# run-house/kubetorch

Measured on NVIDIA H100. Metric: parallel_map_arg_plus_result_GBps, higher is better.
Workload: dtype f32

## Files before the change

### kubetorch_b200/csrc/ktb_map.cu

```cuda
#include "ktb_common.cuh"

#include <algorithm>
#include <atomic>

namespace ktb {

extern int g_red_ctas_per_sm;
extern int g_red_loads;
extern int g_red_fold;
extern int g_seg_large;
extern int g_mlp_chunk_rows;
}
extern int g_mlp_stage_ce;
namespace ktb {
extern std::atomic<int> g_host_zero_copy;
}
extern std::atomic<int> g_push_scatter_ctas_per_sm;
extern std::atomic<int> g_push_slice;
namespace ktb {

static std::atomic<int> g_vec_ctas_per_sm{0};
static std::atomic<int> g_tma_ctas_per_sm{1};
static std::atomic<int> g_tma_cfg{0};
static std::atomic<int> g_auto_variant{KTB_VARIANT_VEC};
static std::atomic<int> g_vec_flavor{2};
static std::atomic<int> g_vec_unroll{4};

constexpr int kVecThreads = 256;
constexpr int kVecUnroll = 4;
constexpr int kVecFlavor = 2;

template <int VB, int FL>
__device__ __forceinline__ void ld_vec(const uint8_t* p, uint32_t (&w)[VB / 4]) {
  static_assert(VB == 16, "sm_90 has no wider per-thread global access than 128 bits");
  if constexpr (FL == 1) {
    asm volatile("ld.global.v4.b32 {%0,%1,%2,%3}, [%4];"
                 : "=r"(w[0]), "=r"(w[1]), "=r"(w[2]), "=r"(w[3])
                 : "l"(p)
                 : "memory");
  } else if constexpr (FL == 2 || FL == 3) {
    ldg128_stream(p, w);
  } else {
    ldg128(p, w);
  }
}
template <int VB, int FL>
__device__ __forceinline__ void st_vec(uint8_t* p, const uint32_t (&w)[VB / 4]) {
  static_assert(VB == 16, "sm_90 has no wider per-thread global access than 128 bits");
  if constexpr (FL == 1) {
    asm volatile("st.global.v4.b32 [%0], {%1,%2,%3,%4};" ::"l"(p), "r"(w[0]), "r"(w[1]), "r"(w[2]), "r"(w[3])
                 : "memory");
  } else if constexpr (FL == 2) {
    stg128_stream(p, w);
  } else {
    stg128(p, w);
  }
}

template <int DT, int OP, int VB, int FL = kVecFlavor, int UNROLL = kVecUnroll>
__global__ void __launch_bounds__(kVecThreads)
    map_vec_kernel(const uint8_t* src, uint8_t* dst, size_t n_bytes, MapParams p) {
  constexpr int NW = VB / 4;
  constexpr int kVecUnroll = UNROLL;
  constexpr size_t TILE = (size_t)kVecThreads * kVecUnroll * VB;
  constexpr size_t ROW = (size_t)kVecThreads * VB;
  const size_t n_full = n_bytes / TILE;

  for (size_t t = blockIdx.x; t < n_full; t += gridDim.x) {
    const size_t off = t * TILE + (size_t)threadIdx.x * VB;
    uint32_t w[kVecUnroll][NW];
#pragma unroll
    for (int j = 0; j < kVecUnroll; ++j) ld_vec<VB, FL>(src + off + j * ROW, w[j]);
#pragma unroll
    for (int j = 0; j < kVecUnroll; ++j) {
      apply_words<DT, OP, NW>(w[j], p);
      st_vec<VB, FL>(dst + off + j * ROW, w[j]);
    }
  }

// ... 76 lines not shown
        }
        fence_proxy_async_smem();
        __syncthreads();
      }
      if (threadIdx.x == 0) {
        bulk_s2g(dst + tile_off(k), buf + (size_t)s * STAGE_BYTES, len);
        bulk_commit();
        if (k >= 1 && (k - 1 + STAGES) < my_n) {
          bulk_wait_read<1>();
          const size_t kn = k - 1 + STAGES;
          const int sn = (int)((k - 1) % STAGES);
          const uint32_t ln = tile_len(kn);
          mbar_expect_tx(&full[sn], ln);
          bulk_g2s(buf + (size_t)sn * STAGE_BYTES, src + tile_off(kn), ln, &full[sn]);
        }
      }
    }
    if (threadIdx.x == 0) bulk_wait_all<0>();
  }

  if (blockIdx.x == 0) {
    constexpr size_t ES = (DT == KTB_U8) ? 1 : ((DT == KTB_BF16 || DT == KTB_F16) ? 2 : (DT == KTB_I64 ? 8 : 4));
    const size_t n_tail = (n_bytes - n16) / ES;
    for (size_t e = threadIdx.x; e < n_tail; e += NT)
      apply_elem<DT, OP>(src + n16 + e * ES, dst + n16 + e * ES, p);
  }
}

template <int DT, int OP>
static int launch_typed(int dev, const uint8_t* src, uint8_t* dst, size_t n_elems, size_t es,
                        const MapParams& p, int variant, cudaStream_t stream) {
  const DeviceInfo* di = device_info(dev);
  const size_t n_bytes = n_elems * es;
  const uintptr_t both = (uintptr_t)src | (uintptr_t)dst;

  if (variant == KTB_VARIANT_AUTO) variant = g_auto_variant.load();
  if (variant == KTB_VARIANT_TMA && (both & 15)) variant = KTB_VARIANT_VEC;
  if (variant == KTB_VARIANT_VEC && (both & 15)) variant = KTB_VARIANT_SCALAR;

  if (variant == KTB_VARIANT_VEC) {
    const int per_sm = g_vec_ctas_per_sm.load();
    auto grid_for = [&](size_t tile_bytes) {
      size_t tiles = std::max<size_t>(n_bytes / tile_bytes, 1);
      if (per_sm <= 0) return (int)std::min<size_t>(tiles, 0x7fffffffULL);
      return (int)std::min<size_t>(tiles, (size_t)di->sm_count * per_sm);
    };
    constexpr bool kTunable = (DT == KTB_U8) || (DT == KTB_F32 && OP == KTB_OP_SCALE);
    const int fl = kTunable ? g_vec_flavor.load() : kVecFlavor;
    const int un = kTunable ? g_vec_unroll.load() : kVecUnroll;
#define KTB_VEC16(FL, UN)                                                                          \
  map_vec_kernel<DT, OP, 16, FL, UN>                                                               \
      <<<grid_for((size_t)kVecThreads * (UN)*16), kVecThreads, 0, stream>>>(src, dst, n_bytes, p)
    if constexpr (kTunable) {
      if (un == 2) {
        if (fl == 1) KTB_VEC16(1, 2); else if (fl == 2) KTB_VEC16(2, 2); else if (fl == 3) KTB_VEC16(3, 2); else KTB_VEC16(0, 2);
      } else if (un == 8) {
        if (fl == 1) KTB_VEC16(1, 8); else if (fl == 2) KTB_VEC16(2, 8); else if (fl == 3) KTB_VEC16(3, 8); else KTB_VEC16(0, 8);
      } else {
        if (fl == 1) KTB_VEC16(1, 4); else if (fl == 2) KTB_VEC16(2, 4); else if (fl == 3) KTB_VEC16(3, 4); else KTB_VEC16(0, 4);
      }
    } else {
      (void)fl; (void)un;
      KTB_VEC16(kVecFlavor, kVecUnroll);
    }
#undef KTB_VEC16
  } else if (variant == KTB_VARIANT_TMA) {
    const int cfg = g_tma_cfg.load();
    const int per_sm = std::max(1, g_tma_ctas_per_sm.load());
#define KTB_LAUNCH_TMA(ST, SB, NT)                                                              \
  do {                                                                                          \
    constexpr size_t smem_bytes = (size_t)(ST) * (SB) + (ST) * sizeof(uint64_t);                \
    auto kfn = map_tma_kernel<DT, OP, ST, SB, NT>;                                              \
    KTB_CK(cudaFuncSetAttribute(kfn, cudaFuncAttributeMaxDynamicSharedMemorySize,               \
                                (int)smem_bytes));                                              \
    size_t tiles = ((n_bytes & ~(size_t)15) + (SB)-1) / (SB);                                   \
    int grid = (int)std::min<size_t>(std::max<size_t>(tiles, 1), (size_t)di->sm_count * per_sm); \
    kfn<<<grid, NT, smem_bytes, stream>>>(src, dst, n_bytes, p);                                \
  } while (0)
    if (cfg == 1) {
      KTB_LAUNCH_TMA(6, 32768, 256);
    } else if (cfg == 2) {
      KTB_LAUNCH_TMA(6, 16384, 256);
    } else if (cfg == 3) {
      KTB_LAUNCH_TMA(3, 65536, 512);
    } else {
      KTB_LAUNCH_TMA(4, 32768, 256);
    }
#undef KTB_LAUNCH_TMA
  } else if (variant == KTB_VARIANT_SCALAR) {
    size_t blocks = (n_elems + 255) / 256;
    int grid = (int)std::min<size_t>(std::max<size_t>(blocks, 1), (size_t)di->sm_count * 8);
    map_scalar_kernel<DT, OP><<<grid, 256, 0, stream>>>(src, dst, n_elems, p);
  } else {
    set_error("ktb_map: unknown variant %d", variant);
    return KTB_ERR_ARG;
  }
  KTB_CK(cudaGetLastError());
  return KTB_OK;
}

int launch_map(int dev, int op, int dtype, const void* src_, void* dst_, size_t n_elems,
               const MapParams& p, int variant, cudaStream_t stream) {
  const uint8_t* src = static_cast<const uint8_t*>(src_);
  uint8_t* dst = static_cast<uint8_t*>(dst_);
  const size_t es = dtype_size(dtype);
  KTB_REQUIRE(es != 0, KTB_ERR_ARG, "ktb_map: unknown dtype %d", dtype);
  KTB_REQUIRE(op >= KTB_OP_IDENTITY && op <= KTB_OP_AFFINE, KTB_ERR_ARG, "ktb_map: unknown op %d", op);
  KTB_REQUIRE(!(dtype == KTB_U8 && op != KTB_OP_IDENTITY), KTB_ERR_ARG,
              "ktb_map: KTB_U8 supports KTB_OP_IDENTITY only");
  if (n_elems == 0) return KTB_OK;
  KTB_REQUIRE(src && dst, KTB_ERR_ARG, "ktb_map: null src/dst with n_elems=%zu", n_elems);
  KTB_REQUIRE((((uintptr_t)src | (uintptr_t)dst) & (es - 1)) == 0, KTB_ERR_ARG,
              "ktb_map: src/dst not aligned to the element size %zu", es);
  KTB_REQUIRE(n_elems <= (SIZE_MAX / 8), KTB_ERR_ARG, "ktb_map: n_elems too large");
  if (src != dst) {
    const uint8_t* se = src + n_elems * es;
    const uint8_t* de = dst + n_elems * es;
    KTB_REQUIRE(se <= dst || de <= src, KTB_ERR_ARG, "ktb_map: src and dst partially overlap");
  }

  if (op == KTB_OP_IDENTITY)
    return launch_typed<KTB_U8, KTB_OP_IDENTITY>(dev, src, dst, n_elems * es, 1, p, variant, stream);

#define KTB_CASE(DT)                                                                              \
  case DT:                                                                                        \
    return (op == KTB_OP_SCALE)                                                                   \
               ? launch_typed<DT, KTB_OP_SCALE>(dev, src, dst, n_elems, es, p, variant, stream)   \
               : launch_typed<DT, KTB_OP_AFFINE>(dev, src, dst, n_elems, es, p, variant, stream);
  switch (dtype) {
    KTB_CASE(KTB_F32)
    KTB_CASE(KTB_BF16)
    KTB_CASE(KTB_I32)
    KTB_CASE(KTB_I64)
    KTB_CASE(KTB_F16)
  }
#undef KTB_CASE
  set_error("ktb_map: unsupported dtype/op %d/%d", dtype, op);
  return KTB_ERR_UNSUPPORTED;
}

}

using namespace ktb;

extern "C" {

int ktb_set_tuning(int key, int value) {
  switch (key) {
    case 0: g_vec_ctas_per_sm = value; return KTB_OK;
    case 1: g_tma_ctas_per_sm = value; return KTB_OK;
    case 2: g_tma_cfg = value; return KTB_OK;
    case 4: g_vec_flavor = value; return KTB_OK;
    case 5: g_vec_unroll = value; return KTB_OK;
    case 6: g_red_ctas_per_sm = value > 0 ? value : 4; return KTB_OK;
    case 12: g_seg_large = value ? 1 : 0; return KTB_OK;
    case 13: g_red_loads = value == 4 ? 4 : 8; return KTB_OK;
    case 14: g_red_fold = value ? 1 : 0; return KTB_OK;
    case 20: g_host_zero_copy = value ? 1 : 0; return KTB_OK;
    case 23: g_push_slice = value > 0 ? value : 1; return KTB_OK;
    case 22: g_mlp_stage_ce = value ? 1 : 0; return KTB_OK;
    case 21: g_push_scatter_ctas_per_sm = value > 0 ? value : 0; return KTB_OK;
    case 8:
      KTB_REQUIRE(value > 0 && value % 128 == 0, KTB_ERR_ARG, "ktb_set_tuning: MLP chunk rows must be a multiple of 128");
      g_mlp_chunk_rows = value;
      return KTB_OK;
    case 3:
      KTB_REQUIRE(value >= KTB_VARIANT_VEC && value <= KTB_VARIANT_SCALAR, KTB_ERR_ARG,
                  "ktb_set_tuning: bad auto variant %d", value);
      g_auto_variant = value;
      return KTB_OK;
    default: set_error("ktb_set_tuning: unknown key %d", key); return KTB_ERR_ARG;
  }
}

int ktb_map(int dev, int op, int dtype, const void* src, void* dst, size_t n_elems, double alpha,
            double beta, int variant, uintptr_t stream) {
  int rc = require_device(dev);
  if (rc) return rc;
  KTB_GUARD(dev);
  return launch_map(dev, op, dtype, src, dst, n_elems, make_params(alpha, beta, dtype), variant,
                    reinterpret_cast<cudaStream_t>(stream));
}

int ktb_map_identity_u8(int dev, const void* src, void* dst, size_t nbytes, uintptr_t stream) {
  return ktb_map(dev, KTB_OP_IDENTITY, KTB_U8, src, dst, nbytes, 1.0, 0.0, KTB_VARIANT_AUTO, stream);
}
int ktb_map_scale_f32(int dev, const float* src, float* dst, size_t n, float alpha, uintptr_t stream) {
  return ktb_map(dev, KTB_OP_SCALE, KTB_F32, src, dst, n, alpha, 0.0, KTB_VARIANT_AUTO, stream);
}
int ktb_map_affine_f32(int dev, const float* src, float* dst, size_t n, float alpha, float beta,
                       uintptr_t stream) {
  return ktb_map(dev, KTB_OP_AFFINE, KTB_F32, src, dst, n, alpha, beta, KTB_VARIANT_AUTO, stream);
}
int ktb_map_scale_bf16(int dev, const void* src, void* dst, size_t n, float alpha, uintptr_t stream) {
  return ktb_map(dev, KTB_OP_SCALE, KTB_BF16, src, dst, n, alpha, 0.0, KTB_VARIANT_AUTO, stream);
}
int ktb_map_affine_bf16(int dev, const void* src, void* dst, size_t n, float alpha, float beta,
                        uintptr_t stream) {
  return ktb_map(dev, KTB_OP_AFFINE, KTB_BF16, src, dst, n, alpha, beta, KTB_VARIANT_AUTO, stream);
}

}
```

### kubetorch_b200/csrc/ktb_mlp.cu

```cuda
#include "ktb_common.cuh"

#include <cuda.h>
#include <algorithm>
#include <atomic>
#include <mutex>

namespace ktb {

constexpr int kMlpBlockM = 128;
constexpr int kMlpBlockK = 64;
constexpr int kMlpWgmmaK = 16;
constexpr int kMlpStages = 4;
constexpr int kMlpConsumers = 256;
constexpr int kMlpThreads = kMlpConsumers + 32;
int g_mlp_chunk_rows = 16896;

__device__ __forceinline__ void tma_load_2d(void* smem_dst, const CUtensorMap* map, int c0, int c1, uint64_t* bar) {
  asm volatile(
      "cp.async.bulk.tensor.2d.shared::cluster.global.mbarrier::complete_tx::bytes [%0], [%1, {%3, %4}], [%2];" ::
          "r"(smem_u32(smem_dst)),
      "l"(map), "r"(smem_u32(bar)), "r"(c0), "r"(c1)
      : "memory");
}
__device__ __forceinline__ void prefetch_tensormap(const CUtensorMap* map) {
  asm volatile("prefetch.tensormap [%0];" ::"l"(map) : "memory");
}
__device__ __forceinline__ void mbar_arrive(uint64_t* bar) {
  asm volatile("mbarrier.arrive.shared::cta.b64 _, [%0];" ::"r"(smem_u32(bar)) : "memory");
}
__device__ __forceinline__ void wgmma_fence() { asm volatile("wgmma.fence.sync.aligned;" ::: "memory"); }
__device__ __forceinline__ void wgmma_commit() { asm volatile("wgmma.commit_group.sync.aligned;" ::: "memory"); }
__device__ __forceinline__ void wgmma_wait_all() { asm volatile("wgmma.wait_group.sync.aligned 0;" ::: "memory"); }

__device__ __forceinline__ uint64_t make_smem_desc_sw128(const void* smem_tile) {
  const uint32_t addr = smem_u32(smem_tile);
  uint64_t d = 0;
  d |= (uint64_t)((addr & 0x3FFFFu) >> 4);
  d |= (uint64_t)1 << 16;
  d |= (uint64_t)(1024u >> 4) << 32;
  d |= (uint64_t)1 << 62;
  return d;
}

template <int N>
struct Wgmma;
template <>
struct Wgmma<256> {
  __device__ __forceinline__ static void mma(float (&d)[128], uint64_t adesc, uint64_t bdesc, uint32_t scale_d) {
    asm volatile(
        "{\n"
        ".reg .pred p;\n"
        "setp.ne.b32 p, %130, 0;\n"
        "wgmma.mma_async.sync.aligned.m64n256k16.f32.bf16.bf16 "
        "{%0,%1,%2,%3,%4,%5,%6,%7,%8,%9,%10,%11,%12,%13,%14,%15,%16,%17,%18,%19,%20,%21,%22,%23,%24,%25,%26,%27,%28,%29,%30,%31,%32,%33,%34,%35,%36,%37,%38,%39,%40,%41,%42,%43,%44,%45,%46,%47,%48,%49,%50,%51,%52,%53,%54,%55,%56,%57,%58,%59,%60,%61,%62,%63,%64,%65,%66,%67,%68,%69,%70,%71,%72,%73,%74,%75,%76,%77,%78,%79,%80,%81,%82,%83,%84,%85,%86,%87,%88,%89,%90,%91,%92,%93,%94,%95,%96,%97,%98,%99,%100,%101,%102,%103,%104,%105,%106,%107,%108,%109,%110,%111,%112,%113,%114,%115,%116,%117,%118,%119,%120,%121,%122,%123,%124,%125,%126,%127}, "
        "%128, %129, p, 1, 1, 0, 0;\n"
        "}\n"
        : "+f"(d[0]), "+f"(d[1]), "+f"(d[2]), "+f"(d[3]), "+f"(d[4]), "+f"(d[5]), "+f"(d[6]), "+f"(d[7]), "+f"(d[8]), "+f"(d[9]), "+f"(d[10]), "+f"(d[11]), "+f"(d[12]), "+f"(d[13]), "+f"(d[14]), "+f"(d[15]), "+f"(d[16]), "+f"(d[17]), "+f"(d[18]), "+f"(d[19]), "+f"(d[20]), "+f"(d[21]), "+f"(d[22]), "+f"(d[23]), "+f"(d[24]), "+f"(d[25]), "+f"(d[26]), "+f"(d[27]), "+f"(d[28]), "+f"(d[29]), "+f"(d[30]), "+f"(d[31]), "+f"(d[32]), "+f"(d[33]), "+f"(d[34]), "+f"(d[35]), "+f"(d[36]), "+f"(d[37]), "+f"(d[38]), "+f"(d[39]), "+f"(d[40]), "+f"(d[41]), "+f"(d[42]), "+f"(d[43]), "+f"(d[44]), "+f"(d[45]), "+f"(d[46]), "+f"(d[47]), "+f"(d[48]), "+f"(d[49]), "+f"(d[50]), "+f"(d[51]), "+f"(d[52]), "+f"(d[53]), "+f"(d[54]), "+f"(d[55]), "+f"(d[56]), "+f"(d[57]), "+f"(d[58]), "+f"(d[59]), "+f"(d[60]), "+f"(d[61]), "+f"(d[62]), "+f"(d[63]), "+f"(d[64]), "+f"(d[65]), "+f"(d[66]), "+f"(d[67]), "+f"(d[68]), "+f"(d[69]), "+f"(d[70]), "+f"(d[71]), "+f"(d[72]), "+f"(d[73]), "+f"(d[74]), "+f"(d[75]), "+f"(d[76]), "+f"(d[77]), "+f"(d[78]), "+f"(d[79]), "+f"(d[80]), "+f"(d[81]), "+f"(d[82]), "+f"(d[83]), "+f"(d[84]), "+f"(d[85]), "+f"(d[86]), "+f"(d[87]), "+f"(d[88]), "+f"(d[89]), "+f"(d[90]), "+f"(d[91]), "+f"(d[92]), "+f"(d[93]), "+f"(d[94]), "+f"(d[95]), "+f"(d[96]), "+f"(d[97]), "+f"(d[98]), "+f"(d[99]), "+f"(d[100]), "+f"(d[101]), "+f"(d[102]), "+f"(d[103]), "+f"(d[104]), "+f"(d[105]), "+f"(d[106]), "+f"(d[107]), "+f"(d[108]), "+f"(d[109]), "+f"(d[110]), "+f"(d[111]), "+f"(d[112]), "+f"(d[113]), "+f"(d[114]), "+f"(d[115]), "+f"(d[116]), "+f"(d[117]), "+f"(d[118]), "+f"(d[119]), "+f"(d[120]), "+f"(d[121]), "+f"(d[122]), "+f"(d[123]), "+f"(d[124]), "+f"(d[125]), "+f"(d[126]), "+f"(d[127])
        : "l"(adesc), "l"(bdesc), "r"(scale_d));
  }
};

template <>
struct Wgmma<64> {
  __device__ __forceinline__ static void mma(float (&d)[32], uint64_t adesc, uint64_t bdesc, uint32_t scale_d) {
    asm volatile(
        "{\n"
        ".reg .pred p;\n"
        "setp.ne.b32 p, %34, 0;\n"
        "wgmma.mma_async.sync.aligned.m64n64k16.f32.bf16.bf16 "
        "{%0,%1,%2,%3,%4,%5,%6,%7,%8,%9,%10,%11,%12,%13,%14,%15,%16,%17,%18,%19,%20,%21,%22,%23,%24,%25,%26,%27,%28,%29,%30,%31}, "
        "%32, %33, p, 1, 1, 0, 0;\n"
        "}\n"
        : "+f"(d[0]), "+f"(d[1]), "+f"(d[2]), "+f"(d[3]), "+f"(d[4]), "+f"(d[5]), "+f"(d[6]), "+f"(d[7]), "+f"(d[8]), "+f"(d[9]), "+f"(d[10]), "+f"(d[11]), "+f"(d[12]), "+f"(d[13]), "+f"(d[14]), "+f"(d[15]), "+f"(d[16]), "+f"(d[17]), "+f"(d[18]), "+f"(d[19]), "+f"(d[20]), "+f"(d[21]), "+f"(d[22]), "+f"(d[23]), "+f"(d[24]), "+f"(d[25]), "+f"(d[26]), "+f"(d[27]), "+f"(d[28]), "+f"(d[29]), "+f"(d[30]), "+f"(d[31])
        : "l"(adesc), "l"(bdesc), "r"(scale_d));
  }
};
template <int BLOCK_N, int STAGES>
struct MlpSmem {
  static constexpr int kABytes = kMlpBlockM * kMlpBlockK * 2;
  static constexpr int kBBytes = BLOCK_N * kMlpBlockK * 2;
  static constexpr int kStageBytes = kABytes + kBBytes;
  static constexpr int kBarrierOff = STAGES * kStageBytes;
  static constexpr int kTotal = kBarrierOff + 2 * STAGES * 8 + 1024 ;
};

template <int BLOCK_N, int STAGES, bool RELU>
__global__ void __launch_bounds__(kMlpThreads, 1)
    gemm_bf16_tn_wgmma_kernel(const __grid_constant__ CUtensorMap map_a, const __grid_constant__ CUtensorMap map_b,
                              __nv_bfloat16* __restrict__ C, int ldc, int K) {
  using S = MlpSmem<BLOCK_N, STAGES>;
  extern __shared__ uint8_t smem_raw[];
  uint8_t* smem = reinterpret_cast<uint8_t*>((reinterpret_cast<uintptr_t>(smem_raw) + 1023) & ~(uintptr_t)1023);
  uint64_t* full = reinterpret_cast<uint64_t*>(smem + S::kBarrierOff);
  uint64_t* empty = full + STAGES;

  const int warp = threadIdx.x >> 5;
  const int lane = threadIdx.x & 31;
  const int n0 = blockIdx.x * BLOCK_N;
  const int m0 = blockIdx.y * kMlpBlockM;
  const int num_kb = K / kMlpBlockK;

  if (threadIdx.x == 0) {
#pragma unroll
    for (int s = 0; s < STAGES; ++s) {
      mbar_init(&full[s], 1);
      mbar_init(&empty[s], kMlpConsumers);
    }
    fence_barrier_init();
  }
  __syncthreads();

  if (warp == kMlpConsumers / 32) {
    if (lane == 0) {
      prefetch_tensormap(&map_a);
      prefetch_tensormap(&map_b);
      for (int kb = 0; kb < num_kb; ++kb) {
        const int s = kb % STAGES;
        mbar_wait(&empty[s], ((kb / STAGES) & 1) ^ 1);
        uint8_t* a_dst = smem + (size_t)s * S::kStageBytes;
        mbar_expect_tx(&full[s], S::kStageBytes);
        tma_load_2d(a_dst, &map_a, kb * kMlpBlockK, m0, &full[s]);
        tma_load_2d(a_dst + S::kABytes, &map_b, kb * kMlpBlockK, n0, &full[s]);
      }
    }
    return;
  }

  const int wg = warp >> 2;
  float acc[BLOCK_N / 2];
#pragma unroll
  for (int i = 0; i < BLOCK_N / 2; ++i) acc[i] = 0.f;
  for (int kb = 0; kb < num_kb; ++kb) {
    const int s = kb % STAGES;
    mbar_wait(&full[s], (kb / STAGES) & 1);
    const uint8_t* a_src = smem + (size_t)s * S::kStageBytes + wg * 64 * 128;
    const uint64_t adesc = make_smem_desc_sw128(a_src);
    const uint64_t bdesc = make_smem_desc_sw128(smem + (size_t)s * S::kStageBytes + S::kABytes);
    wgmma_fence();
#pragma unroll
    for (int k = 0; k < kMlpBlockK / kMlpWgmmaK; ++k) {
      Wgmma<BLOCK_N>::mma(acc, adesc + (uint64_t)(2 * k), bdesc + (uint64_t)(2 * k), (uint32_t)((kb | k) != 0));
    }
    wgmma_commit();
    wgmma_wait_all();
    mbar_arrive(&empty[s]);
  }

  const int row = m0 + wg * 64 + (warp & 3) * 16 + (lane >> 2);
  __nv_bfloat16* c0 = C + (size_t)row * ldc + n0 + 2 * (lane & 3);
  __nv_bfloat16* c1 = c0 + (size_t)8 * ldc;
#pragma unroll
  for (int j = 0; j < BLOCK_N / 8; ++j) {
    float v[4] = {acc[4 * j], acc[4 * j + 1], acc[4 * j + 2], acc[4 * j + 3]};
    if (RELU) {
#pragma unroll
      for (int q = 0; q < 4; ++q) v[q] = fmaxf(v[q], 0.f);
    }
    *reinterpret_cast<__nv_bfloat162*>(c0 + 8 * j) = __floats2bfloat162_rn(v[0], v[1]);
    *reinterpret_cast<__nv_bfloat162*>(c1 + 8 * j) = __floats2bfloat162_rn(v[2], v[3]);
  }
}

typedef CUresult (*PFN_tensorMapEncodeTiled)(CUtensorMap*, CUtensorMapDataType, cuuint32_t, void*, const cuuint64_t*,
                                             const cuuint64_t*, const cuuint32_t*, const cuuint32_t*,
                                             CUtensorMapInterleave, CUtensorMapSwizzle, CUtensorMapL2promotion,
                                             CUtensorMapFloatOOBfill);
static PFN_tensorMapEncodeTiled g_encode = nullptr;
static std::once_flag g_encode_once;

static int get_encoder() {
  std::call_once(g_encode_once, [] {
    void* fn = nullptr;
    cudaDriverEntryPointQueryResult qres;
    if (cudaGetDriverEntryPoint("cuTensorMapEncodeTiled", &fn, cudaEnableDefault, &qres) == cudaSuccess &&
        qres == cudaDriverEntryPointSuccess)
      g_encode = reinterpret_cast<PFN_tensorMapEncodeTiled>(fn);
  });
  KTB_REQUIRE(g_encode != nullptr, KTB_ERR_CUDA, "cuTensorMapEncodeTiled is not available from the driver");
  return KTB_OK;
}

static int encode_map(CUtensorMap* map, const void* base, uint64_t rows, uint64_t cols, uint32_t box_rows);

static int make_map(CUtensorMap* map, const void* base, uint64_t rows, uint64_t cols, uint32_t box_rows) {
  struct Key {
    const void* base;
    uint64_t rows, cols;
    uint32_t box;
    bool operator==(const Key& o) const { return base == o.base && rows == o.rows && cols == o.cols && box == o.box; }
  };
  struct Slot {
    Key key;
    CUtensorMap map;
    bool used = false;
  };
  constexpr int kSlots = 64;
  thread_local Slot cache[kSlots];
  const Key k{base, rows, cols, box_rows};
  const size_t h = ((uintptr_t)base >> 8) * 0x9E3779B97F4A7C15ull + rows * 31 + cols * 7 + box_rows;
  Slot& s = cache[h % kSlots];
  if (s.used && s.key == k) {
    *map = s.map;
    return KTB_OK;
  }
  int rc = encode_map(map, base, rows, cols, box_rows);
  if (rc) return rc;
  s.key = k;
  s.map = *map;
  s.used = true;
  return KTB_OK;
}

static int encode_map(CUtensorMap* map, const void* base, uint64_t rows, uint64_t cols, uint32_t box_rows) {
  cuuint64_t gdim[2] = {cols, rows};
  cuuint64_t gstride[1] = {cols * 2};
  cuuint32_t box[2] = {(cuuint32_t)kMlpBlockK, box_rows};
  cuuint32_t estr[2] = {1, 1};
  CUresult r = g_encode(map, CU_TENSOR_MAP_DATA_TYPE_BFLOAT16, 2, const_cast<void*>(base), gdim, gstride, box, estr,
                        CU_TENSOR_MAP_INTERLEAVE_NONE, CU_TENSOR_MAP_SWIZZLE_128B, CU_TENSOR_MAP_L2_PROMOTION_L2_256B,
                        CU_TENSOR_MAP_FLOAT_OOB_FILL_NONE);
  KTB_REQUIRE(r == CUDA_SUCCESS, KTB_ERR_CUDA, "cuTensorMapEncodeTiled failed with CUresult %d", (int)r);
  return KTB_OK;
}

template <typename KernelT>
static int ensure_smem_attr(KernelT kfn, int smem_bytes, std::atomic<unsigned>& done_mask, int dev) {
  if (dev >= 0 && dev < 32 && (done_mask.load(std::memory_order_acquire) & (1u << dev))) return KTB_OK;
  cudaError_t e = cudaFuncSetAttribute(kfn, cudaFuncAttributeMaxDynamicSharedMemorySize, smem_bytes);
  if (e != cudaSuccess) {
    set_error("cudaFuncSetAttribute(max dynamic shared memory = %d) failed: %s", smem_bytes, cudaGetErrorString(e));
    return KTB_ERR_CUDA;
  }
  if (dev >= 0 && dev < 32) done_mask.fetch_or(1u << dev, std::memory_order_release);
  return KTB_OK;
}

template <int BLOCK_N, bool RELU>
static int launch_gemm(int dev, const void* A, const void* B, void* C, size_t M, int N, int K, int ldc,
                       cudaStream_t stream) {
  using S = MlpSmem<BLOCK_N, kMlpStages>;
  static_assert(S::kTotal <= 232448, "the TMA ring must fit the 227 KiB a block may own");
  CUtensorMap ma, mb;
  int rc = make_map(&ma, A, M, (uint64_t)K, kMlpBlockM);
  if (rc) return rc;
  rc = make_map(&mb, B, (uint64_t)N, (uint64_t)K, BLOCK_N);
  if (rc) return rc;
  auto kfn = gemm_bf16_tn_wgmma_kernel<BLOCK_N, kMlpStages, RELU>;
  static std::atomic<unsigned> attr_done{0};
  rc = ensure_smem_attr(kfn, S::kTotal, attr_done, dev);
  if (rc) return rc;
  dim3 grid((unsigned)(N / BLOCK_N), (unsigned)(M / kMlpBlockM));
  kfn<<<grid, kMlpThreads, S::kTotal, stream>>>(ma, mb, static_cast<__nv_bfloat16*>(C), ldc, K);
  KTB_CK(cudaGetLastError());
  return KTB_OK;
}
}

using namespace ktb;

extern "C" {

size_t ktb_mlp_scratch_bytes(size_t M, int d_hidden) {
  const size_t rows = std::min<size_t>(M, (size_t)g_mlp_chunk_rows);
  return 2 * rows * (size_t)d_hidden * 2;
}

size_t ktb_mlp_stage_bytes(size_t M, int d_in) {
  const size_t rows = std::min<size_t>(M, (size_t)g_mlp_chunk_rows);
  return 2 * rows * (size_t)d_in * 2;
}

int g_mlp_stage_ce = 0;

static int mlp_run(int dev, const void* obs, size_t M, int d_in, int d_hidden, int d_out, const void* W1,
                   const void* W2, const void* W3, void* logits, void* scratch, void* stage, uintptr_t stream) {
  int rc = require_device(dev);
  if (rc) return rc;
  if (M == 0) return KTB_OK;
  KTB_REQUIRE(obs && W1 && W2 && W3 && logits && scratch, KTB_ERR_ARG, "ktb_mlp_bf16: null argument");
  KTB_REQUIRE(M % kMlpBlockM == 0, KTB_ERR_ARG, "ktb_mlp_bf16: M=%zu must be a multiple of %d", M, kMlpBlockM);
  KTB_REQUIRE(d_in > 0 && d_in % kMlpBlockK == 0, KTB_ERR_ARG, "ktb_mlp_bf16: d_in=%d must be a multiple of 64", d_in);
  KTB_REQUIRE(d_hidden > 0 && d_hidden % 256 == 0, KTB_ERR_ARG, "ktb_mlp_bf16: d_hidden=%d must be a multiple of 256",
              d_hidden);
  KTB_REQUIRE(d_out == 64, KTB_ERR_UNSUPPORTED, "ktb_mlp_bf16: d_out=%d (this build carries the 64-wide head)", d_out);
  KTB_REQUIRE((((uintptr_t)obs | (uintptr_t)W1 | (uintptr_t)W2 | (uintptr_t)W3 | (uintptr_t)logits |
                (uintptr_t)scratch | (uintptr_t)stage) & 15) == 0,
              KTB_ERR_ARG, "ktb_mlp_bf16: all pointers must be 16-byte aligned");
  KTB_REQUIRE(g_mlp_chunk_rows % kMlpBlockM == 0 && g_mlp_chunk_rows > 0, KTB_ERR_ARG, "ktb_mlp_bf16: bad chunk rows");
  rc = get_encoder();
  if (rc) return rc;
  KTB_GUARD(dev);
  DeviceInfo* di = device_info(dev);
  cudaStream_t st = reinterpret_cast<cudaStream_t>(stream);
  cudaStream_t side = di->stream_exec;
  const size_t chunk = std::min<size_t>(M, (size_t)g_mlp_chunk_rows);
  __nv_bfloat16* h1 = static_cast<__nv_bfloat16*>(scratch);
  __nv_bfloat16* h2 = h1 + chunk * (size_t)d_hidden;
  const __nv_bfloat16* x = static_cast<const __nv_bfloat16*>(obs);
  __nv_bfloat16* y = static_cast<__nv_bfloat16*>(logits);
  __nv_bfloat16* stg = static_cast<__nv_bfloat16*>(stage);
  const MapParams ident = make_params(1, 0);
  cudaEvent_t evs[5] = {nullptr, nullptr, nullptr, nullptr, nullptr};
  struct EvGuard {
    cudaEvent_t* e;
    ~EvGuard() {
      for (int i = 0; i < 5; ++i)
        if (e[i]) cudaEventDestroy(e[i]);
    }
  } ev_guard{evs};
  static std::mutex side_mu[kMaxDevices];
  std::unique_lock<std::mutex> side_lock;
  if (stg) {
    side_lock = std::unique_lock<std::mutex>(side_mu[dev]);
    for (int i = 0; i < 5; ++i) KTB_CK(cudaEventCreateWithFlags(&evs[i], cudaEventDisableTiming));
    KTB_CK(cudaEventRecord(evs[0], st));
    KTB_CK(cudaStreamWaitEvent(side, evs[0], 0));
  }
  size_t c = 0;
  for (size_t r0 = 0; r0 < M; r0 += chunk, ++c) {
    const size_t rows = std::min(chunk, M - r0);
    const __nv_bfloat16* a1 = x + r0 * d_in;
    if (stg) {
      const int b = (int)(c & 1);
      __nv_bfloat16* dstb = stg + (size_t)b * chunk * d_in;
      if (c >= 2) KTB_CK(cudaStreamWaitEvent(side, evs[3 + b], 0));
      if (g_mlp_stage_ce) {
        KTB_CK(cudaMemcpyAsync(dstb, a1, rows * (size_t)d_in * 2, cudaMemcpyDefault, side));
      } else {
        rc = launch_map(dev, KTB_OP_IDENTITY, KTB_U8, a1, dstb, rows * (size_t)d_in * 2, ident, KTB_VARIANT_AUTO, side);
        if (rc) return rc;
      }
      KTB_CK(cudaEventRecord(evs[1 + b], side));
      KTB_CK(cudaStreamWaitEvent(st, evs[1 + b], 0));
      a1 = dstb;
    }
    rc = launch_gemm<256, true>(dev, a1, W1, h1, rows, d_hidden, d_in, d_hidden, st);
    if (rc) return rc;
    if (stg) KTB_CK(cudaEventRecord(evs[3 + (int)(c & 1)], st));
    rc = launch_gemm<256, true>(dev, h1, W2, h2, rows, d_hidden, d_hidden, d_hidden, st);
    if (rc) return rc;
    rc = launch_gemm<64, false>(dev, h2, W3, y + r0 * d_out, rows, d_out, d_hidden, d_out, st);
    if (rc) return rc;
  }
  return KTB_OK;
}

namespace ktb {
__global__ void mlp_wait_ready_kernel(const unsigned long long* ready, unsigned long long seq, unsigned int* status) {
  if (threadIdx.x == 0) (void)spin_until(ready, seq, status);
}
__global__ void mlp_ack_kernel(unsigned long long* ack, unsigned long long seq) {
  if (threadIdx.x == 0) {
    __threadfence_system();
    st_release_sys(ack, seq);
  }
}
}

int ktb_mlp_bf16_pushed(int dev, const void* stage_local, size_t stage_stride, size_t M, int d_in, int d_hidden, int d_out,
                        const void* W1, const void* W2, const void* W3, void* logits, void* scratch, void* ctrl_local,
                        void* ctrl_root_peer, int rank, size_t chunk_rows, unsigned long long seq, uintptr_t stream) {
  int rc = require_device(dev);
  if (rc) return rc;
  KTB_REQUIRE(stage_local && ctrl_local && ctrl_root_peer && W1 && W2 && W3 && scratch && (logits || M == 0), KTB_ERR_ARG,
              "ktb_mlp_bf16_pushed: null argument");
  KTB_REQUIRE(rank >= 0 && rank < 16 && seq > 0, KTB_ERR_ARG, "ktb_mlp_bf16_pushed: bad rank/seq");
  KTB_REQUIRE(M % kMlpBlockM == 0, KTB_ERR_ARG, "ktb_mlp_bf16_pushed: M=%zu must be a multiple of %d", M, kMlpBlockM);
  KTB_REQUIRE(chunk_rows > 0 && chunk_rows % kMlpBlockM == 0, KTB_ERR_ARG,
              "ktb_mlp_bf16_pushed: chunk_rows=%zu must be a positive multiple of %d", chunk_rows, kMlpBlockM);
  KTB_REQUIRE(d_in > 0 && d_in % kMlpBlockK == 0 && d_hidden > 0 && d_hidden % 256 == 0, KTB_ERR_ARG,
              "ktb_mlp_bf16_pushed: d_in %% 64 and d_hidden %% 256 must be 0");
  KTB_REQUIRE(d_out == 64, KTB_ERR_UNSUPPORTED, "ktb_mlp_bf16_pushed: d_out=%d (this build carries the 64-wide head)", d_out);
  const size_t n_chunks = (M + chunk_rows - 1) / chunk_rows;
  KTB_REQUIRE(n_chunks <= KTB_PUSH_MAX_CHUNKS, KTB_ERR_ARG, "ktb_mlp_bf16_pushed: %zu chunks exceed %d", n_chunks,
              KTB_PUSH_MAX_CHUNKS);
  KTB_REQUIRE(M * (size_t)d_in * 2 <= stage_stride, KTB_ERR_ARG, "ktb_mlp_bf16_pushed: shard exceeds stage_stride");
  rc = get_encoder();
  if (rc) return rc;
  KTB_GUARD(dev);
  cudaStream_t st = reinterpret_cast<cudaStream_t>(stream);
  uint8_t* cl = static_cast<uint8_t*>(ctrl_local);
  const unsigned long long* ready = reinterpret_cast<const unsigned long long*>(cl + KTB_CTRL_READY);
  unsigned int* status = reinterpret_cast<unsigned int*>(cl + KTB_CTRL_STATUS);
  unsigned long long* ack =
      reinterpret_cast<unsigned long long*>(static_cast<uint8_t*>(ctrl_root_peer) + KTB_CTRL_ACK) + rank;
  const __nv_bfloat16* x =
      reinterpret_cast<const __nv_bfloat16*>(static_cast<const uint8_t*>(stage_local) + (size_t)(seq & 1) * stage_stride);
  __nv_bfloat16* h1 = static_cast<__nv_bfloat16*>(scratch);
  __nv_bfloat16* h2 = h1 + std::min(chunk_rows, M) * (size_t)d_hidden;
  __nv_bfloat16* y = static_cast<__nv_bfloat16*>(logits);
  size_t c = 0;
  for (size_t r0 = 0; r0 < M; r0 += chunk_rows, ++c) {
    const size_t rows = std::min(chunk_rows, M - r0);
    mlp_wait_ready_kernel<<<1, 32, 0, st>>>(ready + c, seq, status);
    KTB_CK(cudaGetLastError());
    const __nv_bfloat16* a1 = x + r0 * d_in;
    rc = launch_gemm<256, true>(dev, a1, W1, h1, rows, d_hidden, d_in, d_hidden, st);
    if (rc) return rc;
    rc = launch_gemm<256, true>(dev, h1, W2, h2, rows, d_hidden, d_hidden, d_hidden, st);
    if (rc) return rc;
    rc = launch_gemm<64, false>(dev, h2, W3, y + r0 * d_out, rows, d_out, d_hidden, d_out, st);
    if (rc) return rc;
  }
  mlp_ack_kernel<<<1, 32, 0, st>>>(ack, seq);
  KTB_CK(cudaGetLastError());
  return KTB_OK;
}

int ktb_mlp_bf16(int dev, const void* obs, size_t M, int d_in, int d_hidden, int d_out, const void* W1,
                 const void* W2, const void* W3, void* logits, void* scratch, uintptr_t stream) {
  return mlp_run(dev, obs, M, d_in, d_hidden, d_out, W1, W2, W3, logits, scratch, nullptr, stream);
}

int ktb_mlp_bf16_staged(int dev, const void* obs_peer, size_t M, int d_in, int d_hidden, int d_out, const void* W1,
                        const void* W2, const void* W3, void* logits, void* scratch, void* stage, uintptr_t stream) {
  KTB_REQUIRE(stage, KTB_ERR_ARG, "ktb_mlp_bf16_staged: null stage buffer");
  return mlp_run(dev, obs_peer, M, d_in, d_hidden, d_out, W1, W2, W3, logits, scratch, stage, stream);
}

}
```

Before: 2943.

## Add persistent warp-specialized MLP GEMMs with fused head; lower default vec unroll

Adds a persistent, warp-specialized TMA+WGMMA GEMM kernel that writes layer-1 activations through TMA stores. It fuses layer 2 with the output head, using register-sourced WGMMA so the h2 intermediate never goes to global memory. A new tuning key toggles this chain path, which is on by default. Separately, the default unroll for tunable vectorized map kernels drops from 4 to 1, which shrinks per-CTA tiles and raises the grid size. The goal is fewer launches and less intermediate traffic in the MLP, at the cost of more complex kernels and a map-kernel launch geometry with more, smaller blocks.

```diff
diff --git a/kubetorch_b200/csrc/ktb_map.cu b/kubetorch_b200/csrc/ktb_map.cu
--- a/kubetorch_b200/csrc/ktb_map.cu
+++ b/kubetorch_b200/csrc/ktb_map.cu
@@ -12,6 +12,7 @@
 extern int g_mlp_chunk_rows;
 }
 extern int g_mlp_stage_ce;
+extern int g_mlp_chain;
 namespace ktb {
 extern std::atomic<int> g_host_zero_copy;
 }
@@ -24,7 +25,7 @@
 static std::atomic<int> g_tma_cfg{0};
 static std::atomic<int> g_auto_variant{KTB_VARIANT_VEC};
 static std::atomic<int> g_vec_flavor{2};
-static std::atomic<int> g_vec_unroll{4};
+static std::atomic<int> g_vec_unroll{1};
 
 constexpr int kVecThreads = 256;
 constexpr int kVecUnroll = 4;
@@ -207,13 +208,13 @@
   map_vec_kernel<DT, OP, 16, FL, UN>                                                               \
       <<<grid_for((size_t)kVecThreads * (UN)*16), kVecThreads, 0, stream>>>(src, dst, n_bytes, p)
     if constexpr (kTunable) {
-      if (un == 2) {
-        if (fl == 1) KTB_VEC16(1, 2); else if (fl == 2) KTB_VEC16(2, 2); else if (fl == 3) KTB_VEC16(3, 2); else KTB_VEC16(0, 2);
-      } else if (un == 8) {
-        if (fl == 1) KTB_VEC16(1, 8); else if (fl == 2) KTB_VEC16(2, 8); else if (fl == 3) KTB_VEC16(3, 8); else KTB_VEC16(0, 8);
-      } else {
-        if (fl == 1) KTB_VEC16(1, 4); else if (fl == 2) KTB_VEC16(2, 4); else if (fl == 3) KTB_VEC16(3, 4); else KTB_VEC16(0, 4);
-      }
+#define KTB_VEC16_FL(UN)                                                                                    \
+  do {                                                                                                      \
+    if (fl == 1) KTB_VEC16(1, UN); else if (fl == 2) KTB_VEC16(2, UN); else if (fl == 3) KTB_VEC16(3, UN); \
+    else KTB_VEC16(0, UN);                                                                                \
+  } while (0)
+      if (un == 1) KTB_VEC16_FL(1); else if (un == 2) KTB_VEC16_FL(2); else if (un == 8) KTB_VEC16_FL(8); else KTB_VEC16_FL(4);
+#undef KTB_VEC16_FL
     } else {
       (void)fl; (void)un;
       KTB_VEC16(kVecFlavor, kVecUnroll);
@@ -314,6 +315,7 @@
     case 20: g_host_zero_copy = value ? 1 : 0; return KTB_OK;
     case 23: g_push_slice = value > 0 ? value : 1; return KTB_OK;
     case 22: g_mlp_stage_ce = value ? 1 : 0; return KTB_OK;
+    case 26: g_mlp_chain = value ? 1 : 0; return KTB_OK;
     case 21: g_push_scatter_ctas_per_sm = value > 0 ? value : 0; return KTB_OK;
     case 8:
       KTB_REQUIRE(value > 0 && value % 128 == 0, KTB_ERR_ARG, "ktb_set_tuning: MLP chunk rows must be a multiple of 128");
diff --git a/kubetorch_b200/csrc/ktb_mlp.cu b/kubetorch_b200/csrc/ktb_mlp.cu
--- a/kubetorch_b200/csrc/ktb_mlp.cu
+++ b/kubetorch_b200/csrc/ktb_mlp.cu
@@ -13,6 +13,7 @@
 constexpr int kMlpStages = 4;
 constexpr int kMlpConsumers = 256;
 constexpr int kMlpThreads = kMlpConsumers + 32;
+constexpr int kMlpPersistentThreads = kMlpConsumers + 128;
 int g_mlp_chunk_rows = 16896;
 
 __device__ __forceinline__ void tma_load_2d(void* smem_dst, const CUtensorMap* map, int c0, int c1, uint64_t* bar) {
@@ -22,6 +23,12 @@
       "l"(map), "r"(smem_u32(bar)), "r"(c0), "r"(c1)
       : "memory");
 }
+__device__ __forceinline__ void tma_store_2d(const CUtensorMap* map, const void* smem_src, int c0, int c1) {
+  asm volatile("cp.async.bulk.tensor.2d.global.shared::cta.bulk_group [%0, {%2, %3}], [%1];" ::"l"(map),
+               "r"(smem_u32(smem_src)), "r"(c0), "r"(c1)
+               : "memory");
+}
+__device__ __forceinline__ void warpgroup_bar(int wg) { asm volatile("bar.sync %0, 128;" ::"r"(1 + wg) : "memory"); }
 __device__ __forceinline__ void prefetch_tensormap(const CUtensorMap* map) {
   asm volatile("prefetch.tensormap [%0];" ::"l"(map) : "memory");
 }
@@ -31,6 +38,7 @@
 __device__ __forceinline__ void wgmma_fence() { asm volatile("wgmma.fence.sync.aligned;" ::: "memory"); }
 __device__ __forceinline__ void wgmma_commit() { asm volatile("wgmma.commit_group.sync.aligned;" ::: "memory"); }
 __device__ __forceinline__ void wgmma_wait_all() { asm volatile("wgmma.wait_group.sync.aligned 0;" ::: "memory"); }
+__device__ __forceinline__ void wgmma_wait_one() { asm volatile("wgmma.wait_group.sync.aligned 1;" ::: "memory"); }
 
 __device__ __forceinline__ uint64_t make_smem_desc_sw128(const void* smem_tile) {
   const uint32_t addr = smem_u32(smem_tile);
@@ -58,6 +66,18 @@
         : "+f"(d[0]), "+f"(d[1]), "+f"(d[2]), "+f"(d[3]), "+f"(d[4]), "+f"(d[5]), "+f"(d[6]), "+f"(d[7]), "+f"(d[8]), "+f"(d[9]), "+f"(d[10]), "+f"(d[11]), "+f"(d[12]), "+f"(d[13]), "+f"(d[14]), "+f"(d[15]), "+f"(d[16]), "+f"(d[17]), "+f"(d[18]), "+f"(d[19]), "+f"(d[20]), "+f"(d[21]), "+f"(d[22]), "+f"(d[23]), "+f"(d[24]), "+f"(d[25]), "+f"(d[26]), "+f"(d[27]), "+f"(d[28]), "+f"(d[29]), "+f"(d[30]), "+f"(d[31]), "+f"(d[32]), "+f"(d[33]), "+f"(d[34]), "+f"(d[35]), "+f"(d[36]), "+f"(d[37]), "+f"(d[38]), "+f"(d[39]), "+f"(d[40]), "+f"(d[41]), "+f"(d[42]), "+f"(d[43]), "+f"(d[44]), "+f"(d[45]), "+f"(d[46]), "+f"(d[47]), "+f"(d[48]), "+f"(d[49]), "+f"(d[50]), "+f"(d[51]), "+f"(d[52]), "+f"(d[53]), "+f"(d[54]), "+f"(d[55]), "+f"(d[56]), "+f"(d[57]), "+f"(d[58]), "+f"(d[59]), "+f"(d[60]), "+f"(d[61]), "+f"(d[62]), "+f"(d[63]), "+f"(d[64]), "+f"(d[65]), "+f"(d[66]), "+f"(d[67]), "+f"(d[68]), "+f"(d[69]), "+f"(d[70]), "+f"(d[71]), "+f"(d[72]), "+f"(d[73]), "+f"(d[74]), "+f"(d[75]), "+f"(d[76]), "+f"(d[77]), "+f"(d[78]), "+f"(d[79]), "+f"(d[80]), "+f"(d[81]), "+f"(d[82]), "+f"(d[83]), "+f"(d[84]), "+f"(d[85]), "+f"(d[86]), "+f"(d[87]), "+f"(d[88]), "+f"(d[89]), "+f"(d[90]), "+f"(d[91]), "+f"(d[92]), "+f"(d[93]), "+f"(d[94]), "+f"(d[95]), "+f"(d[96]), "+f"(d[97]), "+f"(d[98]), "+f"(d[99]), "+f"(d[100]), "+f"(d[101]), "+f"(d[102]), "+f"(d[103]), "+f"(d[104]), "+f"(d[105]), "+f"(d[106]), "+f"(d[107]), "+f"(d[108]), "+f"(d[109]), "+f"(d[110]), "+f"(d[111]), "+f"(d[112]), "+f"(d[113]), "+f"(d[114]), "+f"(d[115]), "+f"(d[116]), "+f"(d[117]), "+f"(d[118]), "+f"(d[119]), "+f"(d[120]), "+f"(d[121]), "+f"(d[122]), "+f"(d[123]), "+f"(d[124]), "+f"(d[125]), "+f"(d[126]), "+f"(d[127])
         : "l"(adesc), "l"(bdesc), "r"(scale_d));
   }
+  __device__ __forceinline__ static void mma_first(float (&d)[128], uint64_t adesc, uint64_t bdesc) {
+    asm volatile(
+        "{\n"
+        ".reg .pred p;\n"
+        "setp.ne.b32 p, 0, 0;\n"
+        "wgmma.mma_async.sync.aligned.m64n256k16.f32.bf16.bf16 "
+        "{%0,%1,%2,%3,%4,%5,%6,%7,%8,%9,%10,%11,%12,%13,%14,%15,%16,%17,%18,%19,%20,%21,%22,%23,%24,%25,%26,%27,%28,%29,%30,%31,%32,%33,%34,%35,%36,%37,%38,%39,%40,%41,%42,%43,%44,%45,%46,%47,%48,%49,%50,%51,%52,%53,%54,%55,%56,%57,%58,%59,%60,%61,%62,%63,%64,%65,%66,%67,%68,%69,%70,%71,%72,%73,%74,%75,%76,%77,%78,%79,%80,%81,%82,%83,%84,%85,%86,%87,%88,%89,%90,%91,%92,%93,%94,%95,%96,%97,%98,%99,%100,%101,%102,%103,%104,%105,%106,%107,%108,%109,%110,%111,%112,%113,%114,%115,%116,%117,%118,%119,%120,%121,%122,%123,%124,%125,%126,%127}, "
+        "%128, %129, p, 1, 1, 0, 0;\n"
+        "}\n"
+        : "=f"(d[0]), "=f"(d[1]), "=f"(d[2]), "=f"(d[3]), "=f"(d[4]), "=f"(d[5]), "=f"(d[6]), "=f"(d[7]), "=f"(d[8]), "=f"(d[9]), "=f"(d[10]), "=f"(d[11]), "=f"(d[12]), "=f"(d[13]), "=f"(d[14]), "=f"(d[15]), "=f"(d[16]), "=f"(d[17]), "=f"(d[18]), "=f"(d[19]), "=f"(d[20]), "=f"(d[21]), "=f"(d[22]), "=f"(d[23]), "=f"(d[24]), "=f"(d[25]), "=f"(d[26]), "=f"(d[27]), "=f"(d[28]), "=f"(d[29]), "=f"(d[30]), "=f"(d[31]), "=f"(d[32]), "=f"(d[33]), "=f"(d[34]), "=f"(d[35]), "=f"(d[36]), "=f"(d[37]), "=f"(d[38]), "=f"(d[39]), "=f"(d[40]), "=f"(d[41]), "=f"(d[42]), "=f"(d[43]), "=f"(d[44]), "=f"(d[45]), "=f"(d[46]), "=f"(d[47]), "=f"(d[48]), "=f"(d[49]), "=f"(d[50]), "=f"(d[51]), "=f"(d[52]), "=f"(d[53]), "=f"(d[54]), "=f"(d[55]), "=f"(d[56]), "=f"(d[57]), "=f"(d[58]), "=f"(d[59]), "=f"(d[60]), "=f"(d[61]), "=f"(d[62]), "=f"(d[63]), "=f"(d[64]), "=f"(d[65]), "=f"(d[66]), "=f"(d[67]), "=f"(d[68]), "=f"(d[69]), "=f"(d[70]), "=f"(d[71]), "=f"(d[72]), "=f"(d[73]), "=f"(d[74]), "=f"(d[75]), "=f"(d[76]), "=f"(d[77]), "=f"(d[78]), "=f"(d[79]), "=f"(d[80]), "=f"(d[81]), "=f"(d[82]), "=f"(d[83]), "=f"(d[84]), "=f"(d[85]), "=f"(d[86]), "=f"(d[87]), "=f"(d[88]), "=f"(d[89]), "=f"(d[90]), "=f"(d[91]), "=f"(d[92]), "=f"(d[93]), "=f"(d[94]), "=f"(d[95]), "=f"(d[96]), "=f"(d[97]), "=f"(d[98]), "=f"(d[99]), "=f"(d[100]), "=f"(d[101]), "=f"(d[102]), "=f"(d[103]), "=f"(d[104]), "=f"(d[105]), "=f"(d[106]), "=f"(d[107]), "=f"(d[108]), "=f"(d[109]), "=f"(d[110]), "=f"(d[111]), "=f"(d[112]), "=f"(d[113]), "=f"(d[114]), "=f"(d[115]), "=f"(d[116]), "=f"(d[117]), "=f"(d[118]), "=f"(d[119]), "=f"(d[120]), "=f"(d[121]), "=f"(d[122]), "=f"(d[123]), "=f"(d[124]), "=f"(d[125]), "=f"(d[126]), "=f"(d[127])
+        : "l"(adesc), "l"(bdesc));
+  }
 };
 
 template <>
@@ -74,6 +94,18 @@
         : "+f"(d[0]), "+f"(d[1]), "+f"(d[2]), "+f"(d[3]), "+f"(d[4]), "+f"(d[5]), "+f"(d[6]), "+f"(d[7]), "+f"(d[8]), "+f"(d[9]), "+f"(d[10]), "+f"(d[11]), "+f"(d[12]), "+f"(d[13]), "+f"(d[14]), "+f"(d[15]), "+f"(d[16]), "+f"(d[17]), "+f"(d[18]), "+f"(d[19]), "+f"(d[20]), "+f"(d[21]), "+f"(d[22]), "+f"(d[23]), "+f"(d[24]), "+f"(d[25]), "+f"(d[26]), "+f"(d[27]), "+f"(d[28]), "+f"(d[29]), "+f"(d[30]), "+f"(d[31])
         : "l"(adesc), "l"(bdesc), "r"(scale_d));
   }
+  __device__ __forceinline__ static void mma_rs(float (&d)[32], const uint32_t (&a)[4], uint64_t bdesc, uint32_t scale_d) {
+    asm volatile(
+        "{\n"
+        ".reg .pred p;\n"
+        "setp.ne.b32 p, %37, 0;\n"
+        "wgmma.mma_async.sync.aligned.m64n64k16.f32.bf16.bf16 "
+        "{%0,%1,%2,%3,%4,%5,%6,%7,%8,%9,%10,%11,%12,%13,%14,%15,%16,%17,%18,%19,%20,%21,%22,%23,%24,%25,%26,%27,%28,%29,%30,%31}, "
+        "{%32,%33,%34,%35}, %36, p, 1, 1, 0;\n"
+        "}\n"
+        : "+f"(d[0]), "+f"(d[1]), "+f"(d[2]), "+f"(d[3]), "+f"(d[4]), "+f"(d[5]), "+f"(d[6]), "+f"(d[7]), "+f"(d[8]), "+f"(d[9]), "+f"(d[10]), "+f"(d[11]), "+f"(d[12]), "+f"(d[13]), "+f"(d[14]), "+f"(d[15]), "+f"(d[16]), "+f"(d[17]), "+f"(d[18]), "+f"(d[19]), "+f"(d[20]), "+f"(d[21]), "+f"(d[22]), "+f"(d[23]), "+f"(d[24]), "+f"(d[25]), "+f"(d[26]), "+f"(d[27]), "+f"(d[28]), "+f"(d[29]), "+f"(d[30]), "+f"(d[31])
+        : "r"(a[0]), "r"(a[1]), "r"(a[2]), "r"(a[3]), "l"(bdesc), "r"(scale_d));
+  }
 };
 template <int BLOCK_N, int STAGES>
 struct MlpSmem {
@@ -159,6 +191,176 @@
     *reinterpret_cast<__nv_bfloat162*>(c0 + 8 * j) = __floats2bfloat162_rn(v[0], v[1]);
     *reinterpret_cast<__nv_bfloat162*>(c1 + 8 * j) = __floats2bfloat162_rn(v[2], v[3]);
   }
+}
+
+template <bool FIRST>
+__device__ __forceinline__ void issue_kblock(float (&acc)[128], const uint8_t* stage, int wg) {
+  const uint64_t adesc = make_smem_desc_sw128(stage + wg * 64 * 128);
+  const uint64_t bdesc = make_smem_desc_sw128(stage + kMlpBlockM * kMlpBlockK * 2);
+  wgmma_fence();
+  if (FIRST)
+    Wgmma<256>::mma_first(acc, adesc, bdesc);
+  else
+    Wgmma<256>::mma(acc, adesc, bdesc, 1u);
+#pragma unroll
+  for (int k = 1; k < kMlpBlockK / kMlpWgmmaK; ++k)
+    Wgmma<256>::mma(acc, adesc + (uint64_t)(2 * k), bdesc + (uint64_t)(2 * k), 1u);
+  wgmma_commit();
+}
+
+template <int STAGES, bool FUSE_HEAD>
+struct PersistentSmem {
+  using Ring = MlpSmem<256, STAGES>;
+  static constexpr int kBoxBytes = 64 * kMlpBlockK * 2;
+  static constexpr int kAuxOff = Ring::kBarrierOff;
+  static constexpr int kAuxBytes = (FUSE_HEAD ? 4 : 8) * kBoxBytes;
+  static constexpr int kBarrierOff = kAuxOff + kAuxBytes;
+  static constexpr int kTotal = kBarrierOff + (2 * STAGES + 2) * 8 + 1024 ;
+};
+
+template <int STAGES, bool FUSE_HEAD>
+__global__ void __launch_bounds__(kMlpPersistentThreads, 1)
+    gemm_bf16_tn_persistent_kernel(const __grid_constant__ CUtensorMap map_a, const __grid_constant__ CUtensorMap map_b,
+                                   const __grid_constant__ CUtensorMap map_aux ,
+                                   __nv_bfloat16* __restrict__ C, int ldc, int M, int N, int K) {
+  using S = PersistentSmem<STAGES, FUSE_HEAD>;
+  using Ring = typename S::Ring;
+  extern __shared__ uint8_t smem_raw[];
+  uint8_t* smem = reinterpret_cast<uint8_t*>((reinterpret_cast<uintptr_t>(smem_raw) + 1023) & ~(uintptr_t)1023);
+  uint64_t* full = reinterpret_cast<uint64_t*>(smem + S::kBarrierOff);
+  uint64_t* empty = full + STAGES;
+  uint64_t* head_full = empty + STAGES;
+  uint64_t* head_empty = head_full + 1;
+  uint8_t* head_w = smem + S::kAuxOff;
+
+  const int warp = threadIdx.x >> 5;
+  const int lane = threadIdx.x & 31;
+  const int num_kb = K / kMlpBlockK;
+  const int n_tiles = N / 256;
+  const int units = FUSE_HEAD ? M / kMlpBlockM : (M / kMlpBlockM) * n_tiles;
+  const int tiles_per_unit = FUSE_HEAD ? n_tiles : 1;
+
+  if (threadIdx.x == 0) {
+#pragma unroll
+    for (int s = 0; s < STAGES; ++s) {
+      mbar_init(&full[s], 1);
+      mbar_init(&empty[s], kMlpConsumers);
+    }
+    mbar_init(head_full, 1);
+    mbar_init(head_empty, kMlpConsumers);
+    fence_barrier_init();
+  }
+  __syncthreads();
+
+  if (warp >= kMlpConsumers / 32) {
+    asm volatile("setmaxnreg.dec.sync.aligned.u32 40;\n" ::: "memory");
+    if (warp == kMlpConsumers / 32 && lane == 0) {
+      prefetch_tensormap(&map_a);
+      prefetch_tensormap(&map_b);
+      prefetch_tensormap(&map_aux);
+      uint32_t it = 0, ht = 0;
+      for (int u = blockIdx.x; u < units; u += gridDim.x) {
+        for (int t = 0; t < tiles_per_unit; ++t) {
+          const int m0 = (FUSE_HEAD ? u : u / n_tiles) * kMlpBlockM;
+          const int n0 = (FUSE_HEAD ? t : u % n_tiles) * 256;
+          for (int kb = 0; kb < num_kb; ++kb, ++it) {
+            const int s = it % STAGES;
+            mbar_wait(&empty[s], ((it / STAGES) & 1) ^ 1);
+            uint8_t* a_dst = smem + (size_t)s * Ring::kStageBytes;
+            mbar_expect_tx(&full[s], Ring::kStageBytes);
+            tma_load_2d(a_dst, &map_a, kb * kMlpBlockK, m0, &full[s]);
+            tma_load_2d(a_dst + Ring::kABytes, &map_b, kb * kMlpBlockK, n0, &full[s]);
+          }
+          if (FUSE_HEAD) {
+            mbar_wait(head_empty, (ht & 1) ^ 1);
+            mbar_expect_tx(head_full, S::kAuxBytes);
+#pragma unroll
+            for (int q = 0; q < 4; ++q)
+              tma_load_2d(head_w + q * S::kBoxBytes, &map_aux, n0 + q * kMlpBlockK, 0, head_full);
+            ++ht;
+          }
+        }
+      }
+    }
+    return;
+  }
+
+  asm volatile("setmaxnreg.inc.sync.aligned.u32 232;\n" ::: "memory");
+  const int wg = warp >> 2;
+  const int r_in = wg * 64 + (warp & 3) * 16 + (lane >> 2);
+  float acc[128];
+  float logit[32];
+  uint32_t it = 0, ht = 0;
+  for (int u = blockIdx.x; u < units; u += gridDim.x) {
+    const int m0 = (FUSE_HEAD ? u : u / n_tiles) * kMlpBlockM;
+    for (int t = 0; t < tiles_per_unit; ++t) {
+      const int n0 = (FUSE_HEAD ? t : u % n_tiles) * 256;
+      mbar_wait(&full[it % STAGES], (it / STAGES) & 1);
+      issue_kblock<true>(acc, smem + (size_t)(it % STAGES) * Ring::kStageBytes, wg);
+      ++it;
+      for (int kb = 1; kb < num_kb; ++kb, ++it) {
+        mbar_wait(&full[it % STAGES], (it / STAGES) & 1);
+        issue_kblock<false>(acc, smem + (size_t)(it % STAGES) * Ring::kStageBytes, wg);
+        wgmma_wait_one();
+        mbar_arrive(&empty[(it - 1) % STAGES]);
+      }
+      wgmma_wait_all();
+      mbar_arrive(&empty[(it - 1) % STAGES]);
+
+      if (!FUSE_HEAD) {
+        uint8_t* ctile = head_w + wg * 4 * S::kBoxBytes;
+        const bool leader = (threadIdx.x & 127) == 0;
+        if (leader) bulk_wait_read<0>();
+        warpgroup_bar(wg);
+        const int rl = (warp & 3) * 16 + (lane >> 2);
+#pragma unroll
+        for (int j = 0; j < 32; ++j) {
+          uint8_t* p = ctile + (j >> 3) * S::kBoxBytes + rl * 128 + (((j & 7) ^ (rl & 7)) << 4) + 4 * (lane & 3);
+          *reinterpret_cast<__nv_bfloat162*>(p) =
+              __floats2bfloat162_rn(fmaxf(acc[4 * j], 0.f), fmaxf(acc[4 * j + 1], 0.f));
+          *reinterpret_cast<__nv_bfloat162*>(p + 8 * 128) =
+              __floats2bfloat162_rn(fmaxf(acc[4 * j + 2], 0.f), fmaxf(acc[4 * j + 3], 0.f));
+        }
+        fence_proxy_async_smem();
+        warpgroup_bar(wg);
+        if (leader) {
+#pragma unroll
+          for (int q = 0; q < 4; ++q) tma_store_2d(&map_aux, ctile + q * S::kBoxBytes, n0 + q * 64, m0 + wg * 64);
+          bulk_commit();
+        }
+      } else {
+        uint32_t frag[64];
+#pragma unroll
+        for (int p = 0; p < 64; ++p) {
+          __nv_bfloat162 h2 = __floats2bfloat162_rn(fmaxf(acc[2 * p], 0.f), fmaxf(acc[2 * p + 1], 0.f));
+          frag[p] = *reinterpret_cast<uint32_t*>(&h2);
+        }
+        mbar_wait(head_full, ht & 1);
+        const uint64_t wdesc = make_smem_desc_sw128(head_w);
+        wgmma_fence();
+#pragma unroll
+        for (int kk = 0; kk < 16; ++kk) {
+          const uint32_t a[4] = {frag[4 * kk], frag[4 * kk + 1], frag[4 * kk + 2], frag[4 * kk + 3]};
+          const uint64_t d = wdesc + (uint64_t)((kk >> 2) * (S::kBoxBytes >> 4) + 2 * (kk & 3));
+          Wgmma<64>::mma_rs(logit, a, d, (uint32_t)((t | kk) != 0));
+        }
+        wgmma_commit();
+        wgmma_wait_all();
+        mbar_arrive(head_empty);
+        ++ht;
+      }
+    }
+    if (FUSE_HEAD) {
+      __nv_bfloat16* c0 = C + (size_t)(m0 + r_in) * ldc + 2 * (lane & 3);
+      __nv_bfloat16* c1 = c0 + (size_t)8 * ldc;
+#pragma unroll
+      for (int j = 0; j < 8; ++j) {
+        *reinterpret_cast<__nv_bfloat162*>(c0 + 8 * j) = __floats2bfloat162_rn(logit[4 * j], logit[4 * j + 1]);
+        *reinterpret_cast<__nv_bfloat162*>(c1 + 8 * j) = __floats2bfloat162_rn(logit[4 * j + 2], logit[4 * j + 3]);
+      }
+    }
+  }
+  if (!FUSE_HEAD && (threadIdx.x & 127) == 0) bulk_wait_all<0>();
 }
 
 typedef CUresult (*PFN_tensorMapEncodeTiled)(CUtensorMap*, CUtensorMapDataType, cuuint32_t, void*, const cuuint64_t*,
@@ -254,6 +456,55 @@
   KTB_CK(cudaGetLastError());
   return KTB_OK;
 }
+
+template <bool FUSE_HEAD>
+static int launch_persistent(int dev, const void* A, const void* B, const void* W3, void* C, size_t M, int N, int K,
+                             int ldc, cudaStream_t stream) {
+  constexpr int kStages = FUSE_HEAD ? kMlpStages : 3;
+  using S = PersistentSmem<kStages, FUSE_HEAD>;
+  static_assert(S::kTotal <= 232448, "the TMA ring must fit the 227 KiB a block may own");
+  CUtensorMap ma, mb, maux;
+  int rc = make_map(&ma, A, M, (uint64_t)K, kMlpBlockM);
+  if (rc) return rc;
+  rc = make_map(&mb, B, (uint64_t)N, (uint64_t)K, 256);
+  if (rc) return rc;
+  if (FUSE_HEAD)
+    rc = make_map(&maux, W3, 64, (uint64_t)N, 64);
+  else
+    rc = make_map(&maux, C, M, (uint64_t)ldc, 64);
+  if (rc) return rc;
+  auto kfn = gemm_bf16_tn_persistent_kernel<kStages, FUSE_HEAD>;
+  static std::atomic<unsigned> attr_done{0};
+  rc = ensure_smem_attr(kfn, S::kTotal, attr_done, dev);
+  if (rc) return rc;
+  const size_t units = FUSE_HEAD ? M / kMlpBlockM : M / kMlpBlockM * (size_t)(N / 256);
+  const unsigned grid = (unsigned)std::min<size_t>(units, (size_t)device_info(dev)->sm_count);
+  kfn<<<grid, kMlpPersistentThreads, S::kTotal, stream>>>(ma, mb, maux, static_cast<__nv_bfloat16*>(C), ldc, (int)M, N, K);
+  KTB_CK(cudaGetLastError());
+  return KTB_OK;
+}
+}
+
+int g_mlp_chain = 1;
+
+namespace ktb {
+static int mlp_chunk(int dev, const __nv_bfloat16* x, size_t rows, int d_in, int d_hidden, int d_out, const void* W1,
+                     const void* W2, const void* W3, __nv_bfloat16* y, __nv_bfloat16* h1, __nv_bfloat16* h2,
+                     cudaEvent_t after_l1, cudaStream_t st) {
+  int rc;
+  if (g_mlp_chain) {
+    rc = launch_persistent<false>(dev, x, W1, nullptr, h1, rows, d_hidden, d_in, d_hidden, st);
+    if (rc) return rc;
+    if (after_l1) KTB_CK(cudaEventRecord(after_l1, st));
+    return launch_persistent<true>(dev, h1, W2, W3, y, rows, d_hidden, d_hidden, d_out, st);
+  }
+  rc = launch_gemm<256, true>(dev, x, W1, h1, rows, d_hidden, d_in, d_hidden, st);
+  if (rc) return rc;
+  if (after_l1) KTB_CK(cudaEventRecord(after_l1, st));
+  rc = launch_gemm<256, true>(dev, h1, W2, h2, rows, d_hidden, d_hidden, d_hidden, st);
+  if (rc) return rc;
+  return launch_gemm<64, false>(dev, h2, W3, y, rows, d_out, d_hidden, d_out, st);
+}
 }
 
 using namespace ktb;
@@ -334,12 +585,8 @@
       KTB_CK(cudaStreamWaitEvent(st, evs[1 + b], 0));
       a1 = dstb;
     }
-    rc = launch_gemm<256, true>(dev, a1, W1, h1, rows, d_hidden, d_in, d_hidden, st);
-    if (rc) return rc;
-    if (stg) KTB_CK(cudaEventRecord(evs[3 + (int)(c & 1)], st));
-    rc = launch_gemm<256, true>(dev, h1, W2, h2, rows, d_hidden, d_hidden, d_hidden, st);
-    if (rc) return rc;
-    rc = launch_gemm<64, false>(dev, h2, W3, y + r0 * d_out, rows, d_out, d_hidden, d_out, st);
+    rc = mlp_chunk(dev, a1, rows, d_in, d_hidden, d_out, W1, W2, W3, y + r0 * d_out, h1, h2,
+                   stg ? evs[3 + (int)(c & 1)] : nullptr, st);
     if (rc) return rc;
   }
   return KTB_OK;
@@ -394,12 +641,7 @@
     const size_t rows = std::min(chunk_rows, M - r0);
     mlp_wait_ready_kernel<<<1, 32, 0, st>>>(ready + c, seq, status);
     KTB_CK(cudaGetLastError());
-    const __nv_bfloat16* a1 = x + r0 * d_in;
-    rc = launch_gemm<256, true>(dev, a1, W1, h1, rows, d_hidden, d_in, d_hidden, st);
-    if (rc) return rc;
-    rc = launch_gemm<256, true>(dev, h1, W2, h2, rows, d_hidden, d_hidden, d_hidden, st);
-    if (rc) return rc;
-    rc = launch_gemm<64, false>(dev, h2, W3, y + r0 * d_out, rows, d_out, d_hidden, d_out, st);
+    rc = mlp_chunk(dev, x + r0 * d_in, rows, d_in, d_hidden, d_out, W1, W2, W3, y + r0 * d_out, h1, h2, nullptr, st);
     if (rc) return rc;
   }
   mlp_ack_kernel<<<1, 32, 0, st>>>(ack, seq);
```

Result: faster. 2984, median of 6 (+1.4%).
